# ankitkumar93/compute-war

Measured on AMD Instinct MI355X. Metric: GB/s ingested (Skein-512 + LZ4, 64 KiB blocks), higher is better.
Workload: dtype u64; 1 GPU; skein512+lz4, 1048576 x 65536 B uniform-random blocks/GPU in HBM; blocks_per_gpu=1048576, block_bytes=65536, parallelism=block-sharded x1, gather-only RCCL

## Files before the change

### compute_war_amd/csrc/launch_plan.cpp

```cpp
#include "launch_plan.h"

#include <stdarg.h>
#include <stdio.h>
#include <string.h>

namespace cw {

namespace {

constexpr uint32_t kLaneMidBlocks = 22528, kLaneWideBlocks = 98304;
constexpr bool kLtabDefault = true;
constexpr size_t kLaneLeave = 18432;
constexpr uint32_t kLaneShare = 24576, kLaneShareWide = 32768;
constexpr uint32_t kLaneMinSmall = 61440;

constexpr uint32_t kLzfLaneMinBlocks = 12288;
constexpr uint32_t kLzfLaneMinSmall = 28672;
constexpr size_t kLzfBesideRound = 16384;
constexpr size_t kLzfBigBesideMin = 53248, kLzfBigBesideWide = 98304, kLzfBigBesideRound = 8192, kLzfBigBesideRoundMid = 4096, kLzfBigBesideReserveMid = 12288;
constexpr uint32_t kLzfBesideReserve = 16384, kLzfBesideReserveFew = 8192;

template <class T>
T at_most(T v, T cap) { return v < cap ? v : cap; }

// ... 161 lines not shown
        }
    }
    p.links_lds = kLzfTabBytes + ((big ? kChainMax + 16 : n) + 15u) / 16u * 16u + 32u;
    const uint32_t wave_lds = big ? n2 / 8 + 16u : 2 * n2 + ((n + 15u) & ~15u) + 16u;
    p.per_cu = at_most<size_t>((160u * 1024u) / (wave_lds + 64), big ? 20 : 16);
    p.st_cu = at_most<size_t>((160u * 1024u) / (n2 / 8), st_wpc);
    p.chain_kernel = sthread ? LzfChain::sthread : big ? LzfChain::big : LzfChain::small;
    p.chain_lds = sthread ? n2 / 8 : wave_lds;
    p.spin_cap = kn.lzf_share_give_up ? 0u : kShareSpinCap;
    p.rounds_over_batch = !use_lanes || p.beside;
    p.rounds_over_handback = use_lanes;
    return p;
}

HashPlan hash_plan(const HashCall &call, const Knobs &kn)
{
    HashPlan p;
    const int nw = p.state_words = call.state_words;
    const size_t bb = nw ? (size_t)nw * 8 : 64;
    p.grid = (uint32_t)((call.nblocks + kHashThreads - 1) / kHashThreads);
    p.aligned = call.src_mis16 == 0;
    p.ragged = call.block_bytes == 0 || call.block_bytes % bb != 0;
    if (!nw) return p;
    if (call.may_slice && kn.skein_sliced && call.nblocks >= kSlicedMinBlocks && !p.ragged && call.block_bytes / bb + 1 >= kSlicedMinSteps &&
        p.aligned && call.digest_mis16 == 0) {
        p.sliced = true;
        const size_t total = p.total = call.block_bytes / bb + 1, spl = 128 / bb;
        const size_t nsl = kn.skein_nslices ? (size_t)kn.skein_nslices : kSkeinSlices;
        size_t slice_steps = (total + nsl - 1) / nsl;
        p.slice_steps = slice_steps = (slice_steps + spl - 1) / spl * spl;
        p.state_bytes = call.nblocks * (size_t)nw * sizeof(uint64_t);
        for (size_t b = 0; b < total; b += slice_steps) {
            const size_t e = b + slice_steps < total ? b + slice_steps : total;
            const bool interior = nw == 8 && (e - b) % spl == 0 && e + spl <= total - 1;
            p.slices.push_back({b, e, interior});
        }
        return p;
    }
    const bool steps = kn.skein_mode == SkeinMode::steps;
    p.form = p.ragged ? SkeinForm::ragged : p.aligned && steps ? SkeinForm::steps : SkeinForm::lines;
    return p;
}

namespace {
__attribute__((format(printf, 2, 3))) void add(Description &d, const char *fmt, ...)
{
    const size_t used = strlen(d.text);
    if (used && used + 3 < sizeof d.text) strcat(d.text, " + ");
    const size_t at = strlen(d.text);
    va_list ap;
    va_start(ap, fmt);
    vsnprintf(d.text + at, sizeof d.text - at, fmt, ap);
    va_end(ap);
}
void add_once(Description &d, const char *name, const char *tag = "")
{
    char part[sizeof d.text];
    const size_t len = (size_t)snprintf(part, sizeof part, "%s%s", name, tag);
    if (strstr(d.text, part)) return;
    const size_t used = strlen(d.text);
    if (used + len + 4 < sizeof d.text) { if (used) strcat(d.text, " + "); strcat(d.text, part); }
}
const char *side_tag(const Stage &s) { return s.stream == Target::caller ? "" : " [side stream]"; }
}

Description describe(const Lz4Plan &p)
{
// ... 129 lines not shown
```

### compute_war_amd/csrc/launch_plan.h

```cpp
#pragma once

#include <stddef.h>
#include <stdint.h>
#include <stdlib.h>

#include <string>
#include <vector>

#include "knobs.h"

namespace cw {

constexpr uint32_t kTabBytes = (1u << 13) * 2;
constexpr uint32_t kStageMax = 16384;
constexpr uint32_t kFpBytes = (1u << 13) / 2;
constexpr uint32_t kChunk = 4096;
constexpr uint32_t kLzfTabBytes = (1u << 16) * 2;
constexpr uint32_t kInLdsMax = 16384;
constexpr uint32_t kChainMax = 16384;
constexpr uint32_t kShareSpinCap = 1u << 20;

enum class Lz4ScanSpan : uint8_t { unaligned, aligned };
enum class Lz4Parse : uint8_t { global, staged, fp8, fp16, fp32 };
enum class Lz4Lanes : uint8_t { plain, tagged, fp };
enum class Lz4Ring : uint8_t { k1, k2, k4, k8 };
enum class Lz4Blocks : uint8_t { global, staged };
enum class Lz4Vtab : uint8_t { gen2, gen3, lds_table };
enum class LzfLanes : uint8_t { plain, tagged };
enum class LzfChain : uint8_t { small, big, sthread };
enum class LzfParse : uint8_t { global, staged };

template <class E, class Fn>
struct KernelRow { E id; const char *name; Fn *fn; };
template <class E, class Fn, size_t N>
inline const KernelRow<E, Fn> &kernel_row(const KernelRow<E, Fn> (&table)[N], E id)
{
    for (const auto &r : table)
        if (r.id == id) return r;
    abort();
}
const char *kernel_name(Lz4ScanSpan k);
const char *kernel_name(Lz4Parse k);
const char *kernel_name(Lz4Lanes k);
const char *kernel_name(Lz4Ring k);
const char *kernel_name(Lz4Blocks k);
const char *kernel_name(Lz4Vtab k);
const char *kernel_name(LzfLanes k);
const char *kernel_name(LzfChain k);
const char *kernel_name(LzfParse k);
// ... 54 lines not shown
struct LzfPlan {
    enum class Path : uint8_t { rounds, parse, cut };
    Path path = Path::rounds;
    Stage parse, blocks;
    LzfParse parse_kernel = LzfParse::global;
    uint32_t in_lds = 0, force_redo = 0, blocks_pass = 1;
    bool big = false, beside = false;
    uint32_t n2 = 0;
    size_t chunk = 0, hb_chunk = 0;
    bool rounds_over_batch = false, rounds_over_handback = false;
    LzfChain chain_kernel = LzfChain::small;
    uint32_t links_lds = 0, chain_lds = 0;
    size_t per_cu = 0, st_cu = 0;
    uint32_t spin_cap = 0;
    Stage lanes;
    LzfLanes lanes_kernel = LzfLanes::plain;
    SidePool lanes_pool = SidePool::normal;
    uint32_t lane_reserve = 0;
    size_t links_bytes = 0, lane_tab_bytes = 0, handback_bytes = 0;
};

Lz4Plan lz4_plan(const CodecCall &call, const Knobs &kn, bool lanes_allowed = true);
LzfPlan lzf_plan(const CodecCall &call, const Knobs &kn, bool lanes_allowed = true);

enum class SkeinForm : uint8_t { steps, ragged, lines };
const char *skein_kernel_name(int state_words, SkeinForm form, bool aligned);
const char *skein_slice_kernel_name(int state_words, bool interior);
const char *sha256_kernel_name(bool aligned, bool ragged);

constexpr size_t kHashThreads = 64;
constexpr uint32_t kSkeinSlices = 8;
constexpr size_t kSlicedMinBlocks = 4096;
constexpr size_t kSlicedMinSteps = 256;

struct HashCall {
    int state_words;
    size_t block_bytes, nblocks;
    unsigned src_mis16;
    unsigned digest_mis16;
    bool may_slice;
};
inline HashCall hash_call(int state_words, const void *src, size_t block_bytes, size_t src_stride, size_t nblocks, const void *digests,
                          bool may_slice)
{
    return {state_words, block_bytes, nblocks, (unsigned)((reinterpret_cast<uintptr_t>(src) | src_stride) & 15),
            (unsigned)(reinterpret_cast<uintptr_t>(digests) & 15), may_slice};
}
struct SkeinSlice { size_t begin, end; bool interior; };
struct HashPlan {
    int state_words = 0;
    uint32_t grid = 0;
    bool aligned = false, ragged = false;
    SkeinForm form = SkeinForm::lines;
    bool sliced = false;
    size_t total = 0, slice_steps = 0;
    size_t state_bytes = 0;
    std::vector<SkeinSlice> slices;
};
HashPlan hash_plan(const HashCall &call, const Knobs &kn);

struct Description { char text[320]; };
Description describe(const Lz4Plan &p);
Description describe(const LzfPlan &p);
Description describe(const HashPlan &p);
std::string dump(const Lz4Plan &p);
std::string dump(const LzfPlan &p);
std::string dump(const HashPlan &p);

}
```

### compute_war_amd/csrc/lz4_kernel.hip

```cpp

#include <hip/hip_runtime.h>
#include <stdint.h>
#include <stdio.h>
#include <stdlib.h>
#include <string.h>

#include <optional>
#include <type_traits>

#include "cw_device.h"
#include "lane_codec.h"
#include "launch_plan.h"
#include "lz_device.h"
#include "stream_scratch.h"

#ifndef HEADW_GLOBAL
#define HEADW_GLOBAL 16
#endif
#ifndef HEADW_STAGED
#define HEADW_STAGED 64
#endif

namespace cw {

// ... 95 lines not shown
    }
}

struct BlockFeed {
    size_t next = 0, end = 0;
};
__device__ __forceinline__ bool scan_next_block(BlockFeed &f, size_t &blk, uint32_t *counters, volatile uint32_t *mailbox,
                                                uint32_t run, size_t nblocks, uint32_t lane)
{
    if (f.next == f.end) {
        __syncthreads();
        if (lane == 0) *mailbox = atomicAdd(&counters[2], run);
        __syncthreads();
        f.next = __builtin_amdgcn_readfirstlane(*mailbox);
        f.end = f.next + run;
    }
    blk = f.next++;
    return blk < nblocks;
}

__device__ __forceinline__ void scan_mark(uint32_t *sizes, size_t blk, uint32_t *queue, uint32_t *counters, uint32_t lane)
{
    if (lane == 0) {
        sizes[blk] = kNeedsParse;
        queue[atomicAdd(&counters[1], 1u)] = (uint32_t)blk;
    }
}

__global__ void __launch_bounds__(64)
lz4_scan_kernel(const uint8_t *__restrict__ src, uint32_t n, size_t src_stride, size_t nblocks,
                        uint8_t *__restrict__ dst, size_t dst_stride, uint32_t *__restrict__ sizes, uint32_t nprobes,
                        uint32_t *__restrict__ queue, uint32_t *__restrict__ counters)
{
    __shared__ __attribute__((aligned(16))) uint32_t tab[1u << 13];
    __shared__ __attribute__((aligned(16))) uint32_t mailbox_word[4];
    volatile uint32_t *mailbox = mailbox_word;
    const uint32_t lane = threadIdx.x;
    __builtin_amdgcn_s_setprio(3);
    uint32_t epoch = 15;

    BlockFeed feed;
    const uint32_t run = n >= 65536 ? 1u : 65536u / n;
    for (size_t blk; scan_next_block(feed, blk, counters, mailbox, run, nblocks, lane);) {
        scan_begin_block(tab, epoch, lane);
        const uint8_t *g = src + blk * src_stride;
        uint8_t *out = dst + blk * dst_stride;
        const uint32_t tag = epoch << 28;
        ScanState st;
        bool marked = false;

        if (nprobes) {
            const uint32_t v0 = ld32g(g);
            {
                const uint32_t h0 = v0 * 2654435761u;
                if (lane == 0) atomicMax(&tab[h0 >> 19], tag | ((h0 >> 7) & 0xFFFu));
            }
            for (uint32_t k0 = 0; k0 < nprobes && !marked; k0 += 64 * kScanGroup) {
                uint32_t pos[kScanGroup], v[kScanGroup];
                bool act[kScanGroup];
#pragma unroll
                for (int j = 0; j < kScanGroup; j++) {
                    const uint32_t k = k0 + 64 * j + lane;
                    pos[j] = 1 + probe_delta(k);
                    act[j] = k < nprobes;
                    v[j] = ld32g(g + (act[j] ? pos[j] : 0u));
                }
                uint32_t old[kScanGroup];
#pragma unroll
                for (int j = 0; j < kScanGroup; j++) old[j] = scan_issue(tab, tag, pos[j], v[j], act[j]);
#pragma unroll
                for (int j = 0; j < kScanGroup; j++) scan_judge(old[j], epoch, v0, pos[j], v[j], act[j], st);
                marked = scan_settle(g, st);
            }
        }
        if (marked) {
            scan_mark(sizes, blk, queue, counters, lane);
            continue;
        }
        uint32_t op = 1;
        if (n >= 15) {
            if (lane == 0) out[0] = 15u << 4;
            op += put_len(out + 1, n - 15, lane);
        } else if (lane == 0) {
            out[0] = (uint8_t)(n << 4);
        }
        copy_g2g(out + op, g, n, lane);
        if (lane == 0) sizes[blk] = op + n;
    }
}

constexpr uint32_t kPieces = kChunk / 1024, kRing = 2 * kChunk, kStreamGroup = 2;

struct Chunk { uint4 p[kPieces]; };

__device__ __forceinline__ void chunk_load(Chunk &r, const uint8_t *g, uint32_t c, uint32_t nchunks, uint32_t n, uint32_t lane)
{
#pragma unroll
    for (uint32_t j = 0; j < kPieces; j++) {
        const uint32_t off = c * kChunk + j * 1024 + lane * 16;
        if (c < nchunks && off < n) r.p[j] = *reinterpret_cast<const uint4 *>(g + off);
    }
}
__device__ __forceinline__ void chunk_stage(const Chunk &r, uint32_t *ring32, uint32_t c, uint32_t n, uint32_t lane)
{
#pragma unroll
    for (uint32_t j = 0; j < kPieces; j++) {
        const uint32_t off = c * kChunk + j * 1024 + lane * 16;
        if (off < n) *reinterpret_cast<uint4 *>(reinterpret_cast<uint8_t *>(ring32) + (off & (kRing - 1))) = r.p[j];
    }
}
__device__ __forceinline__ void chunk_store(const Chunk &r, uint8_t *lit, uint32_t c, uint32_t n, uint32_t lane)
{
#pragma unroll
    for (uint32_t j = 0; j < kPieces; j++) {
        const uint32_t off = c * kChunk + j * 1024 + lane * 16;
        if (off < n) {
            uint32_t *q = reinterpret_cast<uint32_t *>(lit + off);
            __builtin_nontemporal_store(r.p[j].x, q);
            __builtin_nontemporal_store(r.p[j].y, q + 1);
            __builtin_nontemporal_store(r.p[j].z, q + 2);
            __builtin_nontemporal_store(r.p[j].w, q + 3);
        }
    }
}
// ... 20 lines not shown
    for (int j = 0; j < NG; j++) scan_judge(old[j], epoch, w.v0, pos[j], v[j], act[j], w.st);
}

__device__ __forceinline__ void probe_upto(Walk &w, uint32_t end, uint32_t *tab, const uint32_t *ring32, uint32_t tag, uint32_t epoch,
                                           uint32_t nprobes, const uint8_t *g, uint32_t lane)
{
    for (;;) {
        uint32_t pos[kStreamGroup], nact = 0, ngroups = 0;
        bool act[kStreamGroup];
#pragma unroll
        for (uint32_t j = 0; j < kStreamGroup; j++) {
            const uint32_t k = w.knext + 64 * j + lane;
            pos[j] = 1 + probe_delta(k);
            act[j] = k < nprobes && pos[j] < end;
            const unsigned long long m = __ballot(act[j]);
            nact += (uint32_t)__builtin_popcountll(m);
            ngroups += m != 0;
        }
        if (nact == 0) return;
        if (ngroups == 1) probe_groups<1>(w, pos, act, tab, ring32, tag, epoch);
        else if (ngroups == 2) probe_groups<2>(w, pos, act, tab, ring32, tag, epoch);
        else probe_groups<kStreamGroup>(w, pos, act, tab, ring32, tag, epoch);
        w.marked = scan_settle(g, w.st);
        w.knext += nact;
        if (w.marked || nact < 64 * kStreamGroup) return;
    }
}

__global__ void __launch_bounds__(64)
lz4_scan_stream_kernel(const uint8_t *__restrict__ src, uint32_t n, size_t src_stride, size_t nblocks,
                       uint8_t *__restrict__ dst, size_t dst_stride, uint32_t *__restrict__ sizes, uint32_t nprobes,
                       uint32_t *__restrict__ queue, uint32_t *__restrict__ counters, size_t first_block, uint32_t feed_word)
{
    __shared__ __attribute__((aligned(16))) uint32_t tab[1u << 13];
    __shared__ __attribute__((aligned(16))) uint32_t ring32[kRing / 4];
    volatile uint32_t *mailbox = ring32;
    const uint32_t lane = threadIdx.x;
    __builtin_amdgcn_s_setprio(3);
    uint32_t epoch = 15;
    const uint32_t nchunks = (n + kChunk - 1) / kChunk;
    const uint32_t hdr = 1 + (n >= 15 ? (n - 15) / 255 + 1 : 0);

    BlockFeed feed;
    const uint32_t run = n >= 65536 ? 1u : 65536u / n;
    for (size_t rel; scan_next_block(feed, rel, counters + feed_word - 2, mailbox, run, nblocks - first_block, lane);) {
        const size_t blk = first_block + rel;
        scan_begin_block(tab, epoch, lane);
        const uint8_t *g = src + blk * src_stride;
        uint8_t *out = dst + blk * dst_stride, *lit = out + hdr;
        const uint32_t tag = epoch << 28;
        Walk w;
        Chunk r0, r1, r2;

#define CW_STAGE(PREV, CUR, C)                                                                         \
        do {                                                                                           \
            const uint32_t c_ = (C);                                                                   \
            if (c_) chunk_store(PREV, lit, c_ - 1, n, lane);                                           \
            chunk_load(PREV, g, c_ + 2, nchunks, n, lane);                                             \
            chunk_stage(CUR, ring32, c_, n, lane);                                                     \
            if (c_ == 0) {                                                                             \
                w.v0 = ring32[0];                                                                      \
                if (nprobes && lane == 0) {                                                            \
                    const uint32_t h0 = w.v0 * 2654435761u;                                            \
                    atomicMax(&tab[h0 >> 19], tag | ((h0 >> 7) & 0xFFFu));             \
                }                                                                                      \
            } else {                                                                                   \
                probe_upto(w, c_ * kChunk, tab, ring32, tag, epoch, nprobes, g, lane);                 \
// ... 44 lines not shown
    uint32_t lo = 0, hi = qlast;
    while (lo < hi) {
        const uint32_t mid = (lo + hi) >> 1;
        if (32 * mid * mid + 32 * mid + 6 <= end) lo = mid + 1;
        else hi = mid;
    }
    return lo;
}

struct SpanWalk {
    uint32_t qnext = 0, v0 = 0;
    bool marked = false;
};

template <int NG, bool PART>
__device__ __forceinline__ bool probe_batches(const uint32_t (&pos)[NG], uint32_t lo, uint32_t hi, uint32_t *tab, const uint32_t *ring32,
                                              uint32_t tag, uint32_t v0, const uint8_t *g, uint32_t lane)
{
    uint32_t v[NG], tp[NG], fp[NG], old[NG];
    const bool act = !PART || (lane >= lo && lane < hi);
    const unsigned long long actm = PART ? __ballot(act) : ~0ull;
#pragma unroll
    for (int j = 0; j < NG; j++) {
        const uint8_t *r8 = reinterpret_cast<const uint8_t *>(ring32);
        const uint32_t wlo = *reinterpret_cast<const uint32_t *>(r8 + (pos[j] & (kRing - 4)));
        const uint32_t whi = *reinterpret_cast<const uint32_t *>(r8 + ((pos[j] + 4) & (kRing - 4)));
        v[j] = __builtin_amdgcn_alignbyte(whi, wlo, pos[j]);
    }
#pragma unroll
    for (int j = 0; j < NG; j++) {
        const uint32_t h = v[j] * 2654435761u;
        fp[j] = (h >> 7) & 0xFFFu;
        tp[j] = tag | (pos[j] << 12);
        old[j] = atomicMax(&tab[act ? h >> 19 : 0u], act ? tp[j] | fp[j] : 0u);
    }
    unsigned long long hit = 0, maybe = 0;
#pragma unroll
    for (int j = 0; j < NG; j++) {
        const unsigned long long empty = __ballot(old[j] < tag);
        hit |= (__ballot(old[j] >= tp[j]) | (empty & __ballot(v[j] == v0))) & actm;
        const unsigned long long fm = __ballot(((old[j] ^ fp[j]) & 0xFFFu) == 0) & ~empty & actm;
        hit |= fm & maybe;
        maybe |= fm;
    }
    if (maybe) {
        uint32_t mcand = 0, mv = 0;
#pragma unroll
        for (int j = 0; j < NG; j++) {
            const bool f = act && old[j] >= tag && ((old[j] ^ fp[j]) & 0xFFFu) == 0;
            mcand = f ? (old[j] >> 12) & 0xFFFFu : mcand;
            mv = f ? v[j] : mv;
        }
        const bool mine = (maybe >> lane) & 1u;
        hit |= __ballot(mine && ld32g(g + mcand) == mv);
    }
    return hit != 0;
}

__device__ __forceinline__ void store16_nt(uint8_t *p, uint32_t x, uint32_t y, uint32_t z, uint32_t w)
{
    typedef uint32_t u32x4 __attribute__((ext_vector_type(4)));
    u32x4 v = {x, y, z, w};
    __builtin_nontemporal_store(v, reinterpret_cast<u32x4 *>(p));
}

__device__ __forceinline__ void probe_partial(SpanWalk &w, uint32_t q, uint32_t nprobes, uint32_t *tab, const uint32_t *ring32, uint32_t tag,
                                              const uint8_t *g, uint32_t lane)
// ... 4 lines not shown
    w.marked = probe_batches<1, true>(pos, q ? 0u : 62u, left < 64 ? left : 64u, tab, ring32, tag, w.v0, g, lane);
    w.qnext = q + 1;
}

__device__ __forceinline__ void probe_range(SpanWalk &w, uint32_t qe, uint32_t *tab, const uint32_t *ring32, uint32_t tag, const uint8_t *g,
                                            uint32_t lane)
{
    uint32_t q = w.qnext;
    w.qnext = qe;
    uint32_t p = __umul24(q, lane) + group_base(q);
    for (; q + 2 <= qe; q += 2) {
        const uint32_t pos[2] = {p, p + lane + (64 * q + 1)};
        if (probe_batches<2, false>(pos, 0, 64, tab, ring32, tag, w.v0, g, lane)) { w.marked = true; return; }
        p = pos[1] + lane + (64 * q + 65);
    }
    if (q < qe) {
        const uint32_t pos[1] = {p};
        w.marked = probe_batches<1, false>(pos, 0, 64, tab, ring32, tag, w.v0, g, lane);
    }
}

#ifdef CW_CLOCK_STAMP
__device__ unsigned long long g_clock_scan[4 * kClockSlots];
hipError_t lz4_clock_read(unsigned long long *out) { return hipMemcpyFromSymbol(out, HIP_SYMBOL(g_clock_scan), sizeof g_clock_scan); }
#endif

template <bool ALIGNED>
__global__ void __launch_bounds__(64)
lz4_scan_span_kernel(const uint8_t *__restrict__ src, uint32_t n, size_t src_stride, uint32_t nspans, uint8_t *__restrict__ dst,
                     size_t dst_stride, uint32_t *__restrict__ sizes, uint32_t nprobes, uint32_t *__restrict__ queue,
                     uint32_t *__restrict__ counters, uint32_t lg)
{
    CW_CLOCK_SCOPE(g_clock_scan);
    __shared__ __attribute__((aligned(16))) uint32_t tab[1u << 13];
    __shared__ __attribute__((aligned(16))) uint32_t ring32[kRing / 4];
    volatile uint32_t *mailbox = ring32;
    const uint32_t lane = threadIdx.x;
    __builtin_amdgcn_s_setprio(3);
    uint32_t epoch = 15;
    const uint32_t cmask = (1u << lg) - 1, run = 16u >> lg;
    const uint32_t hdr = 1 + (n - 15) / 255 + 1;
    const uint32_t lane16 = lane * 16;
    const uint32_t qlast = (nprobes + 61) >> 6;
    const uint32_t gend = group_end((lane + 1) * kChunk < n ? (lane + 1) * kChunk : n, qlast);
    const uint32_t hdrw = (0xFFu << 16) | (((n - 15) % 255) << 24);

    for (;;) {
        __syncthreads();
        if (lane == 0) *mailbox = atomicAdd(&counters[2], 1u);
        __syncthreads();
        const uint32_t span = __builtin_amdgcn_readfirstlane(*mailbox);
        if (span >= nspans) break;
        __syncthreads();
        const size_t first = (size_t)span * run;
        const uint8_t *gs = src + first * src_stride;
        uint8_t *os = dst + first * dst_stride + (ALIGNED ? hdr - 2 : hdr);

        SpanWalk w;
        size_t blk = first;
        uint32_t tag = 0, marks = 0;
        Chunk r0, r1, r2;
#define CW_LD(R, I)                                                                                          \
        do {                                                                                                 \
            const uint32_t i_ = (I) < 15u ? (I) : 15u;                                                       \
            const uint8_t *p_ = gs + (size_t)(i_ >> lg) * src_stride + ((i_ & cmask) << 12) + lane16;        \
            _Pragma("unroll") for (uint32_t j = 0; j < kPieces; j++) R.p[j] = *reinterpret_cast<const uint4 *>(p_ + j * 1024); \
        } while (0)
// ... 1216 lines not shown
const char *kernel_name(Lz4ScanSpan k) { return kernel_row(kScanSpanKernels, k).name; }
const char *kernel_name(Lz4Parse k) { return kernel_row(kParseKernels, k).name; }
const char *kernel_name(Lz4Lanes k) { return kernel_row(kLanesKernels, k).name; }
const char *kernel_name(Lz4Ring k) { return kernel_row(kRingKernels, k).name; }
const char *kernel_name(Lz4Blocks k) { return kernel_row(kBlocksKernels, k).name; }

hipError_t lz4_launch(const uint8_t *src, size_t block_bytes, size_t src_stride, size_t nblocks, uint8_t *dst,
                      size_t dst_stride, uint32_t *sizes, hipStream_t stream, const AfterScan *after_scan)
{
    if (nblocks == 0) return hipSuccess;
    if (!lz4_call_valid(block_bytes, nblocks)) return hipErrorInvalidValue;
    const uint32_t n = (uint32_t)block_bytes;
    const Knobs kn = knobs();
    const CodecCall call = codec_call(src, block_bytes, src_stride, nblocks, dst, dst_stride);
    Lz4Plan p = lz4_plan(call, kn);
    hipError_t e = lz4_set_attributes();
    if (e != hipSuccess) return e;
    auto &wsp = workspaces.at(stream);
    LaunchLock sequence(wsp.launch);
    if ((e = wsp.queues.reserve(p.queue_bytes, p.queue_min_bytes)) != hipSuccess) return e;
    if (p.lanes.on && wsp.lane_tabs.reserve(p.lane_tab_bytes) != hipSuccess) {
        (void)hipGetLastError();
        p = lz4_plan(call, kn, false);
    }
    const size_t cap = (wsp.queues.bytes() / sizeof(uint32_t) - 8) / 2;
    uint32_t *counters = wsp.queues.as<uint32_t>(), *queue = counters + 8, *queue2 = queue + cap;
    uint16_t *const lane_tabs = wsp.lane_tabs.as<uint16_t>();
    std::optional<SideStream::Fork> lanes_fork, vtab_fork;
    auto on = [&](const Stage &s) { return s.stream == Target::lanes_side ? wsp.lanes.stream : s.stream == Target::vtab_side ? wsp.vtab.stream : stream; };
    auto pool = [](SidePool sp) { return sp == SidePool::greatest ? SideStream::greatest : SideStream::normal; };

    if ((e = hipMemsetAsync(counters, 0, 8 * sizeof(uint32_t), stream)) != hipSuccess) return e;
    if (p.scan_span.on)
        hipLaunchKernelGGL(kernel_row(kScanSpanKernels, p.scan_span_kernel).fn, dim3(p.scan_span.grid), dim3(64), 0, stream, src, n, src_stride, p.nspans,
                           dst, dst_stride, sizes, scan_probes(n), queue, counters, p.lg);
    if (p.scan_stream.on)
        hipLaunchKernelGGL(lz4_scan_stream_kernel, dim3(p.scan_stream.grid), dim3(64), 0, stream, src, n, src_stride, nblocks, dst,
                           dst_stride, sizes, scan_probes(n), queue, counters, p.done, 3u);
    if (p.scan_generic.on)
        hipLaunchKernelGGL(lz4_scan_kernel, dim3(p.scan_generic.grid), dim3(64), 0, stream, src, n, src_stride, nblocks, dst,
                           dst_stride, sizes, scan_probes(n), queue, counters);
    if ((e = hipGetLastError()) != hipSuccess) return e;
    if (after_scan && (e = after_scan->fn(after_scan->ctx)) != hipSuccess) return e;
    if (p.stop_after_scan) { note_kernels(0, describe(p).text); return hipSuccess; }
    if (p.lanes.on) {
        if (p.lanes.stream == Target::lanes_side) {
            if ((e = wsp.lanes.open(pool(p.lanes_pool))) != hipSuccess) return e;
            if ((e = lanes_fork.emplace(wsp.lanes, stream).err) != hipSuccess) return e;
        }
        const dim3 lgrid(p.lanes.grid);
        if (p.lanes_form == Lz4Plan::LanesForm::ring_auto)
            hipLaunchKernelGGL(lz4_lanes_ring_auto_kernel, lgrid, dim3(64), 0, on(p.lanes), src, n, src_stride, dst, dst_stride, sizes, queue, counters,
                               lane_tabs, p.lmin, p.reserve, p.wide_from, p.reserve_wide, p.lane_leave);
        else if (p.lanes_form == Lz4Plan::LanesForm::ring)
            hipLaunchKernelGGL(kernel_row(kRingKernels, p.ring_kernel).fn, lgrid, dim3(64), 0, on(p.lanes), src, n, src_stride, dst, dst_stride, sizes, queue,
                               counters, lane_tabs, p.lmin, p.reserve, kNoMax);
        else
            hipLaunchKernelGGL(kernel_row(kLanesKernels, p.lanes_kernel).fn, lgrid, dim3(64), 0, on(p.lanes), src, n, src_stride, dst, dst_stride, sizes, queue,
                               counters, lane_tabs, p.lmin, p.reserve);
        if ((e = hipGetLastError()) != hipSuccess) return e;
    }
    if (p.vtab.on) {
        if (p.vtab.stream == Target::vtab_side) {
            if ((e = wsp.vtab.open(pool(p.vtab_pool))) != hipSuccess) return e;
            if ((e = vtab_fork.emplace(wsp.vtab, stream).err) != hipSuccess) return e;
        }
        if ((e = lz4_vtab_launch(p.vtab_kernel, p.vtab.grid, p.vtab.lds, on(p.vtab), src, n, src_stride, dst, dst_stride, sizes, queue, counters, p.vmin, p.vmax,
                                 p.vres)) != hipSuccess) return e;
    }
    if (p.ltab.on && (e = lz4_vtab_launch(Lz4Vtab::lds_table, p.ltab.grid, p.ltab.lds, stream, src, n, src_stride, dst, dst_stride, sizes, queue, counters, 0u,
                                          kNoMax, 0u)) != hipSuccess) return e;
    if (p.parse.on) {
        hipLaunchKernelGGL(kernel_row(kParseKernels, p.parse_kernel).fn, dim3(p.parse.grid), dim3(64), p.parse.lds, stream, src, n, src_stride, nblocks, dst,
// ... 14 lines not shown
```

### compute_war_amd/csrc/skein_kernels.hip

```cpp

#include <hip/hip_runtime.h>
#include <stdint.h>
#include <stdlib.h>
#include <string.h>

#include "cw_device.h"
#include "launch_plan.h"
#include "stream_scratch.h"

namespace cw {

#define KS_PARITY 0x5555555555555555ULL

template <int R>
static __device__ __forceinline__ uint64_t rotl(uint64_t x)
{
    const uint32_t lo = (uint32_t)x, hi = (uint32_t)(x >> 32);
    uint32_t nlo, nhi;
    if (R == 32) { nlo = hi; nhi = lo; }
    else if (R < 32) {
        nlo = __builtin_amdgcn_alignbit(lo, hi, 32 - R);
        nhi = __builtin_amdgcn_alignbit(hi, lo, 32 - R);
    } else {
        nlo = __builtin_amdgcn_alignbit(hi, lo, 64 - R);
// ... 15 lines not shown
        : "v"((uint32_t)a), "v"((uint32_t)(a >> 32)), "v"((uint32_t)b), "v"((uint32_t)(b >> 32))
        : "vcc");
    return ((uint64_t)hi << 32) | lo;
#else
    return a + b;
#endif
}

#define MIX(a, b, r) do { a = add64(a, b); b = rotl<r>(b) ^ a; } while (0)

#define R512(X, a0, a1, a2, a3, a4, a5, a6, a7, r0, r1, r2, r3) \
    MIX(X[a0], X[a1], r0); MIX(X[a2], X[a3], r1); MIX(X[a4], X[a5], r2); MIX(X[a6], X[a7], r3)

#define INJECT512(X, ks, ts, s)                                              \
    X[0] = add64(X[0], ks[((s) + 0) % 9]); X[1] = add64(X[1], ks[((s) + 1) % 9]); \
    X[2] = add64(X[2], ks[((s) + 2) % 9]); X[3] = add64(X[3], ks[((s) + 3) % 9]); \
    X[4] = add64(X[4], ks[((s) + 4) % 9]);                                   \
    X[5] = add64(add64(X[5], ks[((s) + 5) % 9]), ts[(s) % 3]);               \
    X[6] = add64(add64(X[6], ks[((s) + 6) % 9]), ts[((s) + 1) % 3]);         \
    X[7] = add64(add64(X[7], ks[((s) + 7) % 9]), (uint64_t)(s))

#define EIGHT_ROUNDS_512(X, ks, ts, q)                                       \
    R512(X, 0, 1, 2, 3, 4, 5, 6, 7, 38, 30, 50, 53);                         \
    R512(X, 2, 1, 4, 7, 6, 5, 0, 3, 48, 20, 43, 31);                         \
    R512(X, 4, 1, 6, 3, 0, 5, 2, 7, 34, 14, 15, 27);                         \
    R512(X, 6, 1, 0, 7, 2, 5, 4, 3, 26, 12, 58, 7);                          \
    INJECT512(X, ks, ts, 2 * (q) + 1);                                       \
    R512(X, 0, 1, 2, 3, 4, 5, 6, 7, 33, 49, 8, 42);                          \
    R512(X, 2, 1, 4, 7, 6, 5, 0, 3, 39, 27, 41, 14);                         \
    R512(X, 4, 1, 6, 3, 0, 5, 2, 7, 29, 26, 11, 9);                          \
    R512(X, 6, 1, 0, 7, 2, 5, 4, 3, 33, 51, 39, 35);                         \
    INJECT512(X, ks, ts, 2 * (q) + 2)

static __device__ __forceinline__ void ubi512(uint64_t (&chain)[8], const uint64_t (&w)[8], uint64_t t0, uint64_t t1)
{
    uint64_t ks[9], ts[3], X[8];
    ks[8] = KS_PARITY;
#pragma unroll
    for (int i = 0; i < 8; i++) { ks[i] = chain[i]; ks[8] ^= chain[i]; }
    ts[0] = t0; ts[1] = t1; ts[2] = t0 ^ t1;
#pragma unroll
    for (int i = 0; i < 8; i++) X[i] = add64(w[i], ks[i]);
    X[5] = add64(X[5], ts[0]);
    X[6] = add64(X[6], ts[1]);
    EIGHT_ROUNDS_512(X, ks, ts, 0); EIGHT_ROUNDS_512(X, ks, ts, 1); EIGHT_ROUNDS_512(X, ks, ts, 2);
    EIGHT_ROUNDS_512(X, ks, ts, 3); EIGHT_ROUNDS_512(X, ks, ts, 4); EIGHT_ROUNDS_512(X, ks, ts, 5);
    EIGHT_ROUNDS_512(X, ks, ts, 6); EIGHT_ROUNDS_512(X, ks, ts, 7); EIGHT_ROUNDS_512(X, ks, ts, 8);
#pragma unroll
    for (int i = 0; i < 8; i++) chain[i] = X[i] ^ w[i];
}

#define R256(X, a0, a1, a2, a3, r0, r1) MIX(X[a0], X[a1], r0); MIX(X[a2], X[a3], r1)
#define INJECT256(X, ks, ts, s)                                              \
    X[0] = add64(X[0], ks[((s) + 0) % 5]);                                   \
    X[1] = add64(add64(X[1], ks[((s) + 1) % 5]), ts[(s) % 3]);               \
    X[2] = add64(add64(X[2], ks[((s) + 2) % 5]), ts[((s) + 1) % 3]);         \
    X[3] = add64(add64(X[3], ks[((s) + 3) % 5]), (uint64_t)(s))
#define EIGHT_ROUNDS_256(X, ks, ts, q)                                       \
    R256(X, 0, 1, 2, 3, 5, 56);  R256(X, 0, 3, 2, 1, 36, 28);                \
    R256(X, 0, 1, 2, 3, 13, 46); R256(X, 0, 3, 2, 1, 58, 44);                \
    INJECT256(X, ks, ts, 2 * (q) + 1);                                       \
    R256(X, 0, 1, 2, 3, 26, 20); R256(X, 0, 3, 2, 1, 53, 35);                \
    R256(X, 0, 1, 2, 3, 11, 42); R256(X, 0, 3, 2, 1, 59, 50);                \
    INJECT256(X, ks, ts, 2 * (q) + 2)

static __device__ __forceinline__ void ubi256(uint64_t (&chain)[4], const uint64_t (&w)[4], uint64_t t0, uint64_t t1)
{
    uint64_t ks[5], ts[3], X[4];
    ks[4] = KS_PARITY;
#pragma unroll
    for (int i = 0; i < 4; i++) { ks[i] = chain[i]; ks[4] ^= chain[i]; }
    ts[0] = t0; ts[1] = t1; ts[2] = t0 ^ t1;
#pragma unroll
    for (int i = 0; i < 4; i++) X[i] = add64(w[i], ks[i]);
    X[1] = add64(X[1], ts[0]);
    X[2] = add64(X[2], ts[1]);
    EIGHT_ROUNDS_256(X, ks, ts, 0); EIGHT_ROUNDS_256(X, ks, ts, 1); EIGHT_ROUNDS_256(X, ks, ts, 2);
    EIGHT_ROUNDS_256(X, ks, ts, 3); EIGHT_ROUNDS_256(X, ks, ts, 4); EIGHT_ROUNDS_256(X, ks, ts, 5);
    EIGHT_ROUNDS_256(X, ks, ts, 6); EIGHT_ROUNDS_256(X, ks, ts, 7); EIGHT_ROUNDS_256(X, ks, ts, 8);
#pragma unroll
// ... 167 lines not shown
    fetch_half(A, 0);
    fetch_half(B, HS);

#pragma unroll 1
    for (size_t first = 0; first < total; first += SPL) {
        run_half(A, first);
        fetch_half(A, first + SPL);
        fetch_half(S, first + SPL + HS);
        run_half(B, first + HS);
#pragma unroll
        for (unsigned j = 0; j < HS; j++)
#pragma unroll
            for (int k = 0; k < NW; k++) B[j][k] = S[j][k];
    }

    uint8_t *out = digests + gid * digest_bytes;
    if (((digest_bytes | (unsigned)reinterpret_cast<uintptr_t>(out)) & 15) == 0) {
        uint4 *o4 = reinterpret_cast<uint4 *>(out);
#pragma unroll
        for (int k = 0; k < NW / 2; k++)
            if ((unsigned)(16 * k) < digest_bytes)
                o4[k] = make_uint4((uint32_t)X[2 * k], (uint32_t)(X[2 * k] >> 32), (uint32_t)X[2 * k + 1], (uint32_t)(X[2 * k + 1] >> 32));
    } else {
        for (unsigned k = 0; k < digest_bytes; k++) out[k] = (uint8_t)(X[k >> 3] >> (8 * (k & 7)));
    }
}


#ifdef CW_CLOCK_STAMP
__device__ unsigned long long g_clock_skein[4 * kClockSlots];
hipError_t skein_clock_read(unsigned long long *out) { return hipMemcpyFromSymbol(out, HIP_SYMBOL(g_clock_skein), sizeof g_clock_skein); }
#endif

template <int NW, bool ALIGNED16, bool INTERIOR>
__global__ void __launch_bounds__(CW_SKEIN_THREADS)
skein_slice_kernel(const uint8_t *__restrict__ src, size_t block_bytes, size_t src_stride, size_t nblocks, SkeinIV iv,
                   uint8_t *__restrict__ digests, unsigned digest_bytes, uint64_t *__restrict__ state, size_t s_begin, size_t s_end)
{
    CW_CLOCK_SCOPE_KEYED(g_clock_skein, s_begin / (s_end - s_begin ? s_end - s_begin : 1));
    constexpr unsigned BB = NW * 8, SPL = 128 / BB, HS = SPL / 2;
    const size_t gid = (size_t)blockIdx.x * blockDim.x + threadIdx.x;
    if (gid >= nblocks) return;
    const uint8_t *p = src + gid * src_stride;
    const size_t nmsg = block_bytes / BB, total = nmsg + 1;
    uint64_t *st = state + gid * NW;

    uint64_t X[NW];
    if (s_begin == 0) {
#pragma unroll
        for (int i = 0; i < NW; i++) X[i] = iv.w[i];
    } else {
#pragma unroll
        for (int i = 0; i < NW; i++) X[i] = st[i];
    }
    uint64_t t0 = (uint64_t)s_begin * BB, t1 = (s_begin == 0 ? T1_FIRST : 0) | T1_MSG;

    uint64_t A[HS][NW], B[HS][NW], S[HS][NW];
    auto fetch_half = [&](uint64_t (&dst)[HS][NW], size_t first) __attribute__((always_inline)) {
#pragma unroll
        for (unsigned j = 0; j < HS; j++) {
            const size_t s = first + j;
            if constexpr (INTERIOR) {
                load_words<NW, ALIGNED16>(dst[j], p + s * BB);
            } else {
                const uint64_t keep = s < nmsg ? ~0ull : 0ull;
                load_words<NW, ALIGNED16>(dst[j], p + (s < nmsg ? s : nmsg - 1) * BB);
#pragma unroll
                for (int k = 0; k < NW; k++) dst[j][k] &= keep;
            }
        }
    };
    auto run_half = [&](uint64_t (&buf)[HS][NW], size_t first) {
#pragma unroll
        for (unsigned j = 0; j < HS; j++) {
            const size_t s = first + j;
            if constexpr (INTERIOR) {
                t0 += BB;
                Ubi<NW>::run(X, buf[j], t0, t1);
                t1 &= ~T1_FIRST;
            } else if (s < s_end) {
                if (s + 1 < nmsg) {
                    t0 += BB;
                } else if (s + 1 == nmsg) {
                    t0 += BB;
                    t1 |= T1_FINAL;
                } else {
                    t0 = 8;
                    t1 = T1_FIRST | T1_FINAL | T1_OUT;
                }
                Ubi<NW>::run(X, buf[j], t0, t1);
                t1 &= ~T1_FIRST;
            }
        }
    };
    fetch_half(A, s_begin);
    fetch_half(B, s_begin + HS);
#pragma unroll 1
    for (size_t first = s_begin; first < s_end; first += SPL) {
        run_half(A, first);
        if constexpr (INTERIOR) __builtin_amdgcn_sched_barrier(0);
        fetch_half(A, first + SPL);
        fetch_half(S, first + SPL + HS);
        if constexpr (INTERIOR) __builtin_amdgcn_sched_barrier(0);
        run_half(B, first + HS);
#pragma unroll
        for (unsigned j = 0; j < HS; j++)
#pragma unroll
            for (int k = 0; k < NW; k++) B[j][k] = S[j][k];
    }

    if (INTERIOR || s_end < total) {
#pragma unroll
        for (int i = 0; i < NW; i++) st[i] = X[i];
        return;
    }
    uint8_t *out = digests + gid * digest_bytes;
    if (((digest_bytes | (unsigned)reinterpret_cast<uintptr_t>(out)) & 15) == 0) {
        uint4 *o4 = reinterpret_cast<uint4 *>(out);
#pragma unroll
        for (int k = 0; k < NW / 2; k++)
            if ((unsigned)(16 * k) < digest_bytes)
                o4[k] = make_uint4((uint32_t)X[2 * k], (uint32_t)(X[2 * k] >> 32), (uint32_t)X[2 * k + 1], (uint32_t)(X[2 * k + 1] >> 32));
    } else {
        for (unsigned k = 0; k < digest_bytes; k++) out[k] = (uint8_t)(X[k >> 3] >> (8 * (k & 7)));
    }
}

namespace {
StreamScratch<DeviceBuf> slices;

struct SkeinRow { int nw; SkeinForm form; bool aligned; const char *name; decltype(skein_lines_kernel<8, true>) *fn; };
#define CW_ROW_BLOCKS(NW, A, R) {NW, R ? SkeinForm::ragged : SkeinForm::steps, A, "cw::skein_blocks_kernel<" #NW ", " #A ", " #R ">", skein_blocks_kernel<NW, A, R>}
#define CW_ROW_LINES(NW, A) {NW, SkeinForm::lines, A, "cw::skein_lines_kernel<" #NW ", " #A ">", skein_lines_kernel<NW, A>}
const SkeinRow kSkeinKernels[] = {
    CW_ROW_BLOCKS(8, true, false), CW_ROW_BLOCKS(8, true, true), CW_ROW_BLOCKS(8, false, true), CW_ROW_LINES(8, true), CW_ROW_LINES(8, false),
    CW_ROW_BLOCKS(4, true, false), CW_ROW_BLOCKS(4, true, true), CW_ROW_BLOCKS(4, false, true), CW_ROW_LINES(4, true), CW_ROW_LINES(4, false),
};
#undef CW_ROW_BLOCKS
#undef CW_ROW_LINES
struct SkeinSliceRow { int nw; bool interior; const char *name; decltype(skein_slice_kernel<8, true, true>) *fn; };
const SkeinSliceRow kSkeinSliceKernels[] = {
    {8, true, "cw::skein_slice_kernel<8, true, true>", skein_slice_kernel<8, true, true>},
    {8, false, "cw::skein_slice_kernel<8, true, false>", skein_slice_kernel<8, true, false>},
    {4, false, "cw::skein_slice_kernel<4, true, false>", skein_slice_kernel<4, true, false>},
// ... 271 lines not shown
```

Baseline: 1143 GB/s.

## Specialize Skein interior slice with 32-bit lane offsets and fenced UBI rounds

Splits the interior Skein-512 slice path into its own device function. It uses 32-bit per-lane offsets from a block-wide base pointer, a countdown loop, and scheduling barriers between each eight-round group, so that 64-bit address arithmetic and register pressure stay low. The interior form is turned off when the source stride is too wide for 32-bit lane offsets. Separately, the LZ4 scan kernels move their hash table to dynamic shared memory, and an asm barrier on the atomic slot index constrains how the compiler schedules it. The extra sched barriers could limit instruction interleaving.

```diff
diff --git a/compute_war_amd/csrc/launch_plan.cpp b/compute_war_amd/csrc/launch_plan.cpp
--- a/compute_war_amd/csrc/launch_plan.cpp
+++ b/compute_war_amd/csrc/launch_plan.cpp
@@ -217,7 +217,7 @@
         p.state_bytes = call.nblocks * (size_t)nw * sizeof(uint64_t);
         for (size_t b = 0; b < total; b += slice_steps) {
             const size_t e = b + slice_steps < total ? b + slice_steps : total;
-            const bool interior = nw == 8 && (e - b) % spl == 0 && e + spl <= total - 1;
+            const bool interior = nw == 8 && (e - b) % spl == 0 && e + spl <= total - 1 && !call.wide_stride;
             p.slices.push_back({b, e, interior});
         }
         return p;
diff --git a/compute_war_amd/csrc/launch_plan.h b/compute_war_amd/csrc/launch_plan.h
--- a/compute_war_amd/csrc/launch_plan.h
+++ b/compute_war_amd/csrc/launch_plan.h
@@ -15,6 +15,9 @@
 constexpr uint32_t kStageMax = 16384;
 constexpr uint32_t kFpBytes = (1u << 13) / 2;
 constexpr uint32_t kChunk = 4096;
+constexpr uint32_t kScanTabWords = 1u << 13;
+constexpr uint32_t kScanTabBytes = kScanTabWords * 4;
+constexpr uint32_t kScanRing = 2 * kChunk;
 constexpr uint32_t kLzfTabBytes = (1u << 16) * 2;
 constexpr uint32_t kInLdsMax = 16384;
 constexpr uint32_t kChainMax = 16384;
@@ -135,6 +138,7 @@
 constexpr uint32_t kSkeinSlices = 8;
 constexpr size_t kSlicedMinBlocks = 4096;
 constexpr size_t kSlicedMinSteps = 256;
+constexpr size_t kSkeinLaneStrideMax = 0xFFFFFFFFull / (kHashThreads - 1);
 
 struct HashCall {
     int state_words;
@@ -142,12 +146,13 @@
     unsigned src_mis16;
     unsigned digest_mis16;
     bool may_slice;
+    bool wide_stride = false;
 };
 inline HashCall hash_call(int state_words, const void *src, size_t block_bytes, size_t src_stride, size_t nblocks, const void *digests,
                           bool may_slice)
 {
     return {state_words, block_bytes, nblocks, (unsigned)((reinterpret_cast<uintptr_t>(src) | src_stride) & 15),
-            (unsigned)(reinterpret_cast<uintptr_t>(digests) & 15), may_slice};
+            (unsigned)(reinterpret_cast<uintptr_t>(digests) & 15), may_slice, src_stride > kSkeinLaneStrideMax};
 }
 struct SkeinSlice { size_t begin, end; bool interior; };
 struct HashPlan {
diff --git a/compute_war_amd/csrc/lz4_kernel.hip b/compute_war_amd/csrc/lz4_kernel.hip
--- a/compute_war_amd/csrc/lz4_kernel.hip
+++ b/compute_war_amd/csrc/lz4_kernel.hip
@@ -151,7 +151,7 @@
                         uint8_t *__restrict__ dst, size_t dst_stride, uint32_t *__restrict__ sizes, uint32_t nprobes,
                         uint32_t *__restrict__ queue, uint32_t *__restrict__ counters)
 {
-    __shared__ __attribute__((aligned(16))) uint32_t tab[1u << 13];
+    extern __shared__ __attribute__((aligned(16))) uint32_t tab[];
     __shared__ __attribute__((aligned(16))) uint32_t mailbox_word[4];
     volatile uint32_t *mailbox = mailbox_word;
     const uint32_t lane = threadIdx.x;
@@ -208,7 +208,7 @@
     }
 }
 
-constexpr uint32_t kPieces = kChunk / 1024, kRing = 2 * kChunk, kStreamGroup = 2;
+constexpr uint32_t kPieces = kChunk / 1024, kRing = kScanRing, kStreamGroup = 2;
 
 struct Chunk { uint4 p[kPieces]; };
 
@@ -295,7 +295,7 @@
                        uint8_t *__restrict__ dst, size_t dst_stride, uint32_t *__restrict__ sizes, uint32_t nprobes,
                        uint32_t *__restrict__ queue, uint32_t *__restrict__ counters, size_t first_block, uint32_t feed_word)
 {
-    __shared__ __attribute__((aligned(16))) uint32_t tab[1u << 13];
+    extern __shared__ __attribute__((aligned(16))) uint32_t tab[];
     __shared__ __attribute__((aligned(16))) uint32_t ring32[kRing / 4];
     volatile uint32_t *mailbox = ring32;
     const uint32_t lane = threadIdx.x;
@@ -406,7 +406,9 @@
         const uint32_t h = v[j] * 2654435761u;
         fp[j] = (h >> 7) & 0xFFFu;
         tp[j] = tag | (pos[j] << 12);
-        old[j] = atomicMax(&tab[act ? h >> 19 : 0u], act ? tp[j] | fp[j] : 0u);
+        uint32_t slot = act ? h >> 19 : 0u;
+        asm("" : "+v"(slot));
+        old[j] = atomicMax(&tab[slot], act ? tp[j] | fp[j] : 0u);
     }
     unsigned long long hit = 0, maybe = 0;
 #pragma unroll
@@ -477,7 +479,7 @@
                      uint32_t *__restrict__ counters, uint32_t lg)
 {
     CW_CLOCK_SCOPE(g_clock_scan);
-    __shared__ __attribute__((aligned(16))) uint32_t tab[1u << 13];
+    extern __shared__ __attribute__((aligned(16))) uint32_t tab[];
     __shared__ __attribute__((aligned(16))) uint32_t ring32[kRing / 4];
     volatile uint32_t *mailbox = ring32;
     const uint32_t lane = threadIdx.x;
@@ -1760,13 +1762,13 @@
 
     if ((e = hipMemsetAsync(counters, 0, 8 * sizeof(uint32_t), stream)) != hipSuccess) return e;
     if (p.scan_span.on)
-        hipLaunchKernelGGL(kernel_row(kScanSpanKernels, p.scan_span_kernel).fn, dim3(p.scan_span.grid), dim3(64), 0, stream, src, n, src_stride, p.nspans,
+        hipLaunchKernelGGL(kernel_row(kScanSpanKernels, p.scan_span_kernel).fn, dim3(p.scan_span.grid), dim3(64), kScanTabBytes, stream, src, n, src_stride, p.nspans,
                            dst, dst_stride, sizes, scan_probes(n), queue, counters, p.lg);
     if (p.scan_stream.on)
-        hipLaunchKernelGGL(lz4_scan_stream_kernel, dim3(p.scan_stream.grid), dim3(64), 0, stream, src, n, src_stride, nblocks, dst,
+        hipLaunchKernelGGL(lz4_scan_stream_kernel, dim3(p.scan_stream.grid), dim3(64), kScanTabBytes, stream, src, n, src_stride, nblocks, dst,
                            dst_stride, sizes, scan_probes(n), queue, counters, p.done, 3u);
     if (p.scan_generic.on)
-        hipLaunchKernelGGL(lz4_scan_kernel, dim3(p.scan_generic.grid), dim3(64), 0, stream, src, n, src_stride, nblocks, dst,
+        hipLaunchKernelGGL(lz4_scan_kernel, dim3(p.scan_generic.grid), dim3(64), kScanTabBytes, stream, src, n, src_stride, nblocks, dst,
                            dst_stride, sizes, scan_probes(n), queue, counters);
     if ((e = hipGetLastError()) != hipSuccess) return e;
     if (after_scan && (e = after_scan->fn(after_scan->ctx)) != hipSuccess) return e;
diff --git a/compute_war_amd/csrc/skein_kernels.hip b/compute_war_amd/csrc/skein_kernels.hip
--- a/compute_war_amd/csrc/skein_kernels.hip
+++ b/compute_war_amd/csrc/skein_kernels.hip
@@ -71,8 +71,10 @@
     R512(X, 6, 1, 0, 7, 2, 5, 4, 3, 33, 51, 39, 35);                         \
     INJECT512(X, ks, ts, 2 * (q) + 2)
 
+template <bool FENCED = false>
 static __device__ __forceinline__ void ubi512(uint64_t (&chain)[8], const uint64_t (&w)[8], uint64_t t0, uint64_t t1)
 {
+#define CW_FENCE() do { if constexpr (FENCED) __builtin_amdgcn_sched_barrier(0); } while (0)
     uint64_t ks[9], ts[3], X[8];
     ks[8] = KS_PARITY;
 #pragma unroll
@@ -82,9 +84,11 @@
     for (int i = 0; i < 8; i++) X[i] = add64(w[i], ks[i]);
     X[5] = add64(X[5], ts[0]);
     X[6] = add64(X[6], ts[1]);
-    EIGHT_ROUNDS_512(X, ks, ts, 0); EIGHT_ROUNDS_512(X, ks, ts, 1); EIGHT_ROUNDS_512(X, ks, ts, 2);
-    EIGHT_ROUNDS_512(X, ks, ts, 3); EIGHT_ROUNDS_512(X, ks, ts, 4); EIGHT_ROUNDS_512(X, ks, ts, 5);
-    EIGHT_ROUNDS_512(X, ks, ts, 6); EIGHT_ROUNDS_512(X, ks, ts, 7); EIGHT_ROUNDS_512(X, ks, ts, 8);
+    CW_FENCE();
+    EIGHT_ROUNDS_512(X, ks, ts, 0); CW_FENCE(); EIGHT_ROUNDS_512(X, ks, ts, 1); CW_FENCE(); EIGHT_ROUNDS_512(X, ks, ts, 2); CW_FENCE();
+    EIGHT_ROUNDS_512(X, ks, ts, 3); CW_FENCE(); EIGHT_ROUNDS_512(X, ks, ts, 4); CW_FENCE(); EIGHT_ROUNDS_512(X, ks, ts, 5); CW_FENCE();
+    EIGHT_ROUNDS_512(X, ks, ts, 6); CW_FENCE(); EIGHT_ROUNDS_512(X, ks, ts, 7); CW_FENCE(); EIGHT_ROUNDS_512(X, ks, ts, 8); CW_FENCE();
+#undef CW_FENCE
 #pragma unroll
     for (int i = 0; i < 8; i++) chain[i] = X[i] ^ w[i];
 }
@@ -318,6 +322,63 @@
 hipError_t skein_clock_read(unsigned long long *out) { return hipMemcpyFromSymbol(out, HIP_SYMBOL(g_clock_skein), sizeof g_clock_skein); }
 #endif
 
+template <int NW>
+static __device__ __forceinline__ void skein_slice_interior(const uint8_t *__restrict__ src, size_t src_stride, const SkeinIV &iv,
+                                                            uint64_t *__restrict__ state, size_t s_begin, size_t s_end)
+{
+    constexpr unsigned BB = NW * 8, SPL = 128 / BB, HS = SPL / 2;
+    const size_t first = (size_t)blockIdx.x * CW_SKEIN_THREADS;
+    uint32_t lane_off = threadIdx.x * (uint32_t)src_stride;
+    const uint8_t *line = src + first * src_stride + s_begin * BB;
+    uint64_t *wst = state + first * NW;
+
+    uint64_t X[NW];
+    if (s_begin == 0) {
+#pragma unroll
+        for (int i = 0; i < NW; i++) X[i] = iv.w[i];
+    } else {
+        load_words<NW, true>(X, reinterpret_cast<const uint8_t *>(wst) + threadIdx.x * (NW * 8u));
+    }
+    uint64_t t0 = (uint64_t)s_begin * BB, t1 = (s_begin == 0 ? T1_FIRST : 0) | T1_MSG;
+
+    uint64_t A[HS][NW], B[HS][NW], S[HS][NW];
+    auto fetch_half = [&](uint64_t (&dst)[HS][NW], unsigned at) __attribute__((always_inline)) {
+#pragma unroll
+        for (unsigned j = 0; j < HS; j++) load_words<NW, true>(dst[j], line + (at + j) * BB + lane_off);
+    };
+    auto run_half = [&](uint64_t (&buf)[HS][NW]) {
+#pragma unroll
+        for (unsigned j = 0; j < HS; j++) {
+            t0 += BB;
+            static_assert(NW == 8, "the interior slice is built for Skein-512 only");
+            ubi512<true>(X, buf[j], t0, t1);
+            t1 &= ~T1_FIRST;
+        }
+    };
+    fetch_half(A, 0);
+    fetch_half(B, HS);
+#pragma unroll 1
+    for (uint32_t lines = (uint32_t)((s_end - s_begin) / SPL); lines; lines--) {
+        run_half(A);
+        __builtin_amdgcn_sched_barrier(0);
+        line += 128;
+        asm volatile("" : "+v"(lane_off));
+        fetch_half(A, 0);
+        fetch_half(S, HS);
+        __builtin_amdgcn_sched_barrier(0);
+        run_half(B);
+#pragma unroll
+        for (unsigned j = 0; j < HS; j++)
+#pragma unroll
+            for (int k = 0; k < NW; k++) B[j][k] = S[j][k];
+    }
+
+    const uint32_t lane = __builtin_amdgcn_mbcnt_hi(~0u, __builtin_amdgcn_mbcnt_lo(~0u, 0u));
+    uint64_t *st = reinterpret_cast<uint64_t *>(reinterpret_cast<uint8_t *>(wst) + lane * (NW * 8u));
+#pragma unroll
+    for (int i = 0; i < NW; i++) st[i] = X[i];
+}
+
 template <int NW, bool ALIGNED16, bool INTERIOR>
 __global__ void __launch_bounds__(CW_SKEIN_THREADS)
 skein_slice_kernel(const uint8_t *__restrict__ src, size_t block_bytes, size_t src_stride, size_t nblocks, SkeinIV iv,
@@ -327,6 +388,10 @@
     constexpr unsigned BB = NW * 8, SPL = 128 / BB, HS = SPL / 2;
     const size_t gid = (size_t)blockIdx.x * blockDim.x + threadIdx.x;
     if (gid >= nblocks) return;
+    if constexpr (INTERIOR) {
+        skein_slice_interior<NW>(src, src_stride, iv, state, s_begin, s_end);
+        return;
+    }
     const uint8_t *p = src + gid * src_stride;
     const size_t nmsg = block_bytes / BB, total = nmsg + 1;
     uint64_t *st = state + gid * NW;
@@ -346,25 +411,17 @@
 #pragma unroll
         for (unsigned j = 0; j < HS; j++) {
             const size_t s = first + j;
-            if constexpr (INTERIOR) {
-                load_words<NW, ALIGNED16>(dst[j], p + s * BB);
-            } else {
-                const uint64_t keep = s < nmsg ? ~0ull : 0ull;
-                load_words<NW, ALIGNED16>(dst[j], p + (s < nmsg ? s : nmsg - 1) * BB);
-#pragma unroll
-                for (int k = 0; k < NW; k++) dst[j][k] &= keep;
-            }
+            const uint64_t keep = s < nmsg ? ~0ull : 0ull;
+            load_words<NW, ALIGNED16>(dst[j], p + (s < nmsg ? s : nmsg - 1) * BB);
+#pragma unroll
+            for (int k = 0; k < NW; k++) dst[j][k] &= keep;
         }
     };
     auto run_half = [&](uint64_t (&buf)[HS][NW], size_t first) {
 #pragma unroll
         for (unsigned j = 0; j < HS; j++) {
             const size_t s = first + j;
-            if constexpr (INTERIOR) {
-                t0 += BB;
-                Ubi<NW>::run(X, buf[j], t0, t1);
-                t1 &= ~T1_FIRST;
-            } else if (s < s_end) {
+            if (s < s_end) {
                 if (s + 1 < nmsg) {
                     t0 += BB;
                 } else if (s + 1 == nmsg) {
@@ -384,10 +441,8 @@
 #pragma unroll 1
     for (size_t first = s_begin; first < s_end; first += SPL) {
         run_half(A, first);
-        if constexpr (INTERIOR) __builtin_amdgcn_sched_barrier(0);
         fetch_half(A, first + SPL);
         fetch_half(S, first + SPL + HS);
-        if constexpr (INTERIOR) __builtin_amdgcn_sched_barrier(0);
         run_half(B, first + HS);
 #pragma unroll
         for (unsigned j = 0; j < HS; j++)
@@ -395,7 +450,7 @@
             for (int k = 0; k < NW; k++) B[j][k] = S[j][k];
     }
 
-    if (INTERIOR || s_end < total) {
+    if (s_end < total) {
 #pragma unroll
         for (int i = 0; i < NW; i++) st[i] = X[i];
         return;
```

Measured after the change: 1152 GB/s (median of 6 runs). Within noise of the previous version (+0.8%).
